# zertovitch/zip-ada

Measured on NVIDIA B200. Metric: bzip2_encode_MBps_900k, higher is better.
Workload: dtype u8

## Files before the change

zip-ada_b200/csrc/b2_api.cu:

```cuda
#include "b2_common.cuh"
#include "b2_kernels.h"
#include "../../include/b2gpu.h"

#include <algorithm>
#include <atomic>
#include <cmath>
#include <condition_variable>
#include <cstdlib>
#include <cstring>
#include <deque>
#include <chrono>
#include <map>
#include <mutex>
#include <string>
#include <thread>
#include <vector>
#include <unordered_set>

static thread_local std::string g_last_error = "";
void b2_set_error(const char *file, int line, const char *msg) {
  char buf[512];
  snprintf(buf, sizeof buf, "%s:%d: %s", file, line, msg);
  g_last_error = buf;
}
// ... 117 lines not shown
  DevBuf<u8> d_packed;
  DevBuf<u32> d_cut_first, d_cut_last, d_cut_tsum;
  DevBuf<u64> d_cut_carry, d_cut_tincl;
  DevBuf<u8> d_cut_gs;
  DevBuf<u16> d_cut_gm;
  DevBuf<B2ZipCrcTables> d_zt;
  DevBuf<B2ZipTile> d_ztiles;
  DevBuf<B2ZipEntry> d_zents;
  DevBuf<B2ZipCopy> d_zcopies;
  DevBuf<u32> d_zpartial, d_zcrc;
  DevBuf<u8> d_vstream, d_vlcol, d_vrle, d_vsel;
  DevBuf<u32> d_vlink, d_vchain, d_vscal;
  DevBuf<u64> d_vcand;
  DevBuf<B2VBlock> d_vblocks;
  std::vector<Workspace *> ws;
  std::vector<B2Chunk> chunks;
  std::vector<u32> nseg;
  std::vector<std::vector<u32>> seg;
  std::vector<b2_chunk_trace> trace;
  b2_stats stats;
  B2SortStats sort_stats;
  bool batch_positions_fixed = false;
  size_t batch_positions = 1536ull << 20;
  size_t first_batch_positions = ~(size_t)0;
  size_t batch_jobs_max = 65535;
  int n_workspaces = 1;
  u64 launches_other = 0;
  cudaEvent_t ev[2] = {nullptr, nullptr};
  cudaEvent_t ev_call[2] = {nullptr, nullptr};
};

namespace {

struct StageTimer {
  cudaStream_t st; cudaEvent_t *ev; double *acc; bool on;
  StageTimer(b2_encoder *e, cudaStream_t st_, cudaEvent_t *ev_, double *acc_) : st(st_), ev(ev_), acc(acc_), on(e->timing >= 2) {
    if (on) cudaEventRecord(ev[0], st);
  }
  ~StageTimer() {
    if (on) {
      cudaEventRecord(ev[1], st);
      cudaEventSynchronize(ev[1]);
      float ms = 0; cudaEventElapsedTime(&ms, ev[0], ev[1]);
      *acc += ms;
    }
  }
};

void balance_window(int level, i64 &lo, i64 &hi) {
  volatile float fcap = (float)(100000 * level);
  volatile float flo = fcap * 1.05f, fhi = fcap * 1.30f;
  lo = -1; hi = -2;
  i64 base = 100000ll * level;
  for (i64 v = base; v <= 2 * base; v++) {
    volatile float f = (float)v;
    if (f >= flo && f <= fhi) { if (lo < 0) lo = v; hi = v; }
  }
}

int ensure_batch_workspace(Workspace *w, size_t T, size_t J) {
  const size_t max_tiles = T / B2_SORT_TILE + J + 8;
  const size_t max_mtiles = T / B2_MTF_TILE + J + 8;
  const size_t GT = T / B2_GROUP_SIZE + 20 * J + 32;
  B2_TRY(w->d_scalars.ensure(16));
  B2_TRY(w->d_jobs.ensure(J));
  B2_TRY(w->d_text.ensure(T + 64)); B2_TRY(w->d_bwt.ensure(T + 64)); B2_TRY(w->d_idx.ensure(T + 64));
  B2_TRY(w->d_m16.ensure((T / 16 + 8 * J + 8) * 8)); B2_TRY(w->d_m256.ensure((T / 256 + 2 * J + 8) * 8));
  B2_TRY(w->d_keysA.ensure(T)); B2_TRY(w->d_keysB.ensure(T));
  B2_TRY(w->d_valsA.ensure(T)); B2_TRY(w->d_valsB.ensure(T));
  B2_TRY(w->d_rank.ensure(T)); B2_TRY(w->d_grp.ensure(T));
  B2_TRY(w->d_slotA.ensure(T)); B2_TRY(w->d_slotB.ensure(T)); B2_TRY(w->d_sa.ensure(T)); B2_TRY(w->d_tile_cnt.ensure(max_tiles));
  B2_TRY(w->d_tiles.ensure(max_tiles)); B2_TRY(w->d_tiles_rr.ensure(max_tiles)); B2_TRY(w->d_mtiles.ensure(max_mtiles));
  B2_TRY(w->d_tilemask.ensure(max_mtiles * 8)); B2_TRY(w->d_msegs.ensure(T / B2_MTF_SEG + J + 8));
  B2_TRY(w->d_sj.ensure(J));
  B2_TRY(w->d_hist.ensure(max_tiles * 256)); B2_TRY(w->d_digit_base.ensure(J * 8 * 256 + 256));
  B2_TRY(w->d_tile_head.ensure(max_tiles)); B2_TRY(w->d_carry.ensure(max_tiles));
  B2_TRY(w->d_unsorted.ensure(J));
  B2_TRY(w->d_mtf.ensure(T + 16 * J + 64)); B2_TRY(w->d_ghist.ensure(T + 16 * J + 64));
  B2_TRY(w->d_rank3.ensure(GT)); B2_TRY(w->d_rank4.ensure(GT)); B2_TRY(w->d_gdist.ensure(GT));
  B2_TRY(w->d_sel.ensure(GT * B2_N_TRIPLES + 64)); B2_TRY(w->d_selprev.ensure(GT * B2_N_TRIPLES + 64));
  B2_TRY(w->d_selpos.ensure(GT));
  B2_TRY(w->d_gpack.ensure(GT * B2_N_TRIPLES + 64)); B2_TRY(w->d_gselcost.ensure(GT * B2_N_TRIPLES + 64));
  B2_TRY(w->d_ehist.ensure(J * B2_N_TRIPLES * B2_MAX_CODERS * 260));
  B2_TRY(w->d_leaves.ensure((J * B2_N_TRIPLES * B2_MAX_CODERS + 64) * 260)); B2_TRY(w->d_wl.ensure(J * B2_N_TRIPLES * (B2_MAX_CODERS + 3) + J / 32 + 512));
  B2_TRY(w->d_estat.ensure(J * B2_N_TRIPLES * 2)); B2_TRY(w->d_selcost.ensure(J * B2_N_TRIPLES));
  B2_TRY(w->d_lens.ensure(J * B2_N_TRIPLES * B2_MAX_CODERS * B2_MAX_ALPHA));
  B2_TRY(w->d_cost.ensure(J * B2_N_TRIPLES)); B2_TRY(w->d_low.ensure(J * B2_N_TRIPLES));
  B2_TRY(w->d_items.ensure(J));
  if (J > w->h_unsorted_cap) {
    if (w->h_unsorted) cudaFreeHost(w->h_unsorted);
    B2_CUDA_CHECK(cudaMallocHost((void **)&w->h_unsorted, (J + 64) * sizeof(u32)));
    w->h_unsorted_cap = J + 64;
  }
  return 0;
}

u64 layout_jobs(std::vector<B2Job> &jobs, int level) {
  u64 pos = 0, mpos = 0;
  for (auto &j : jobs) {
    u64 cap = std::min<u64>((u64)j.raw_len * 5 / 4 + 8, (u64)level * 100000 + 64);
    cap = (cap + 255) & ~255ull;
    j.pos_off = (u32)pos; j.cap = (u32)cap;
    pos += cap;
    j.mtf_off = (u32)mpos;
    mpos += (cap + 2 + 7) & ~7ull;
  }
  return pos;
}

int run_batch(b2_encoder *e, Workspace *w, const u8 *d_in, std::vector<B2Job> &jobs) {
  const u32 J = (u32)jobs.size();
  if (J == 0) return 0;
  const u64 T = layout_jobs(jobs, e->level);
  if (T >= (1ull << 32) - (1ull << 20)) B2_FAIL(B2_ERR_INTERNAL, "batch too large for 32-bit arena offsets (lower B2GPU_BATCH_POSITIONS)");
  B2_TRY(ensure_batch_workspace(w, (size_t)T + 64, J));
  cudaStream_t st = w->st;
  B2_CUDA_CHECK(cudaMemcpyAsync(w->d_jobs.p, jobs.data(), J * sizeof(B2Job), cudaMemcpyHostToDevice, st));
  {
    StageTimer tm(e, st, w->ev, &w->stage_ms[1]);
    B2_TRY(b2k_rle1(st, d_in, w->d_jobs.p, J, w->d_text.p, e->d_ct.p));
    w->launches += 1;
  }
  w->batch_jobs.resize(J);
  B2_CUDA_CHECK(cudaMemcpyAsync(w->batch_jobs.data(), w->d_jobs.p, J * sizeof(B2Job), cudaMemcpyDeviceToHost, st));
  B2_CUDA_CHECK(cudaStreamSynchronize(st));
  u32 gpos = 0, max_g = 1;
  std::vector<u32> ids(J), ns(J);
  std::vector<B2SortTile> mtiles, msegs, msegs_mid, msegs_big;
  for (u32 j = 0; j < J; j++) {
    B2Job &b = w->batch_jobs[j];
    if (b.n > b.cap) B2_FAIL(B2_ERR_INTERNAL, "RLE1 output exceeds its slot");
    u32 gmax = (b.n / B2_GROUP_SIZE + 2 + 15) & ~15u;
    b.grp_off = gpos; gpos += gmax;
    max_g = std::max(max_g, gmax);
    ids[j] = j; ns[j] = b.n;
    b.na = b.n;
    b.tile0 = (u32)mtiles.size();
    for (u32 s = 0; s < b.n; s += B2_MTF_TILE) mtiles.push_back(B2SortTile{j, s});
    for (u32 s = 0; s < b.n; s += B2_MTF_SEG) (b.n_used <= 64 ? msegs : b.n_used <= 128 ? msegs_mid : msegs_big).push_back(B2SortTile{j, s});
    w->block_bytes += b.n;
  }
  w->blocks += J;
  w->total_groups = gpos;
  B2_CUDA_CHECK(cudaMemcpyAsync(w->d_jobs.p, w->batch_jobs.data(), J * sizeof(B2Job), cudaMemcpyHostToDevice, st));
  {
    StageTimer tm(e, st, w->ev, &w->stage_ms[2]);
    B2SortCtx cx;
    cx.keysA = w->d_keysA.p; cx.keysB = w->d_keysB.p; cx.valsA = w->d_valsA.p; cx.valsB = w->d_valsB.p;
    cx.rank = w->d_rank.p; cx.grp = w->d_grp.p; cx.d_tiles = w->d_tiles.p; cx.d_sj = w->d_sj.p;
    cx.slotA = w->d_slotA.p; cx.slotB = w->d_slotB.p; cx.sa_full = w->d_sa.p; cx.d_tile_cnt = w->d_tile_cnt.p;
    cx.d_hist = w->d_hist.p; cx.d_digit_base = w->d_digit_base.p; cx.d_tiles_rr = w->d_tiles_rr.p; cx.d_ticket = w->d_digit_base.p + w->d_digit_base.cap - 256; cx.d_tile_head = w->d_tile_head.p; cx.d_carry = w->d_carry.p;
    cx.d_unsorted = w->d_unsorted.p; cx.h_unsorted = w->h_unsorted;
    cx.max_tiles = w->d_tiles.cap; cx.max_jobs = w->d_sj.cap; cx.timing = e->timing >= 1;
    cx.stats = w->sort_stats;
    {
      u32 max_used = 1;
      for (u32 j = 0; j < J; j++) max_used = std::max(max_used, w->batch_jobs[j].n_used);
      cx.sym_bits = 1;
      while ((1u << cx.sym_bits) < max_used) cx.sym_bits++;
      cx.max_used = max_used;
      cx.h_jobs = w->batch_jobs.data();
    }
    if (e->timing >= 1) cudaEventRecord(w->ev_sort[0], st);
    int rc = b2k_bwt_batch(&cx, st, w->d_jobs.p, ids, ns, w->d_text.p, w->d_bwt.p);
    if (e->timing >= 1) cudaEventRecord(w->ev_sort[1], st);
    w->sort_stats = cx.stats;
    if (rc) return rc;
// ... 1326 lines not shown
```

zip-ada_b200/csrc/b2_entropy.cu:

```cuda
#include "b2_common.cuh"
#include "b2_kernels.h"

#define HSTRIDE 260
#define QS_SMALL 100

__global__ void __launch_bounds__(256)
k_group_keys(const B2Job *__restrict__ jobs, const u16 *__restrict__ mtf, u32 *__restrict__ rank3, u32 *__restrict__ rank4) {
  const B2Job &job = jobs[blockIdx.x];
  const u32 M = job.n_mtf, G = job.n_groups;
  const u16 *m = mtf + job.mtf_off;
  const u32 eob = job.n_used + 1;
  const u32 lim3 = eob < 3 ? eob : 3, lim4 = eob < 4 ? eob : 4;
  for (u32 g = threadIdx.x; g < G; g += blockDim.x) {
    u32 s0 = g * B2_GROUP_SIZE, s1 = min(s0 + B2_GROUP_SIZE, M);
    u32 k3 = 0, k4 = 0;
    for (u32 s = s0; s < s1; s++) { u32 sym = m[s]; k3 += sym < lim3; k4 += sym < lim4; }
    rank3[job.grp_off + g] = (k3 << 16) | (g + 1);
    rank4[job.grp_off + g] = (k4 << 16) | (g + 1);
  }
}

__global__ void __launch_bounds__(256)
k_group_hist(const B2Job *__restrict__ jobs, const u16 *__restrict__ mtf, u16 *__restrict__ ghist, u8 *__restrict__ gdist) {
  const B2Job &job = jobs[blockIdx.x];
// ... 32 lines not shown
    }
    cntA += addA;
    const bool newB = leadB && foundAt == 0xFFFFFFFFu;
    const u32 bmB = __ballot_sync(0xffffffffu, newB);
    u16 *e = gh + s0;
    if (leadA) e[slotA] = (u16)((cntA << 9) | symA);
    if (newB) e[DA + __popc(bmB & lt)] = (u16)((cntB << 9) | symB);
    if (l == 0) gdist[job.grp_off + g] = (u8)(DA + __popc(bmB));
  }
}

__global__ void __launch_bounds__(32)
k_rank_sort(const B2Job *__restrict__ jobs, u32 *__restrict__ rank3, u32 *__restrict__ rank4, u32 g_lo, u32 g_hi) {
  extern __shared__ __align__(16) u32 a[];
  const B2Job &job = jobs[blockIdx.x >> 1];
  u32 *arr = ((blockIdx.x & 1) ? rank4 : rank3) + job.grp_off;
  const i32 G = (i32)job.n_groups;
  if ((u32)G <= g_lo || (u32)G > g_hi) return;
  for (i32 i = threadIdx.x; i < G; i += 32) a[i + 1] = arr[i];
  __syncwarp();
  if (threadIdx.x == 0) {
    i32 mx = G;
    u32 temp;
#define KEY(x) ((x) >> 16)
    auto sift = [&](i32 s) {
      i32 c = s;
      while (8 * c + 7 <= mx) {
        const uint2 pr = *reinterpret_cast<const uint2 *>(&a[2 * c]);
        const uint4 qd = *reinterpret_cast<const uint4 *>(&a[4 * c]);
        const uint4 o0 = *reinterpret_cast<const uint4 *>(&a[8 * c]);
        const uint4 o1 = *reinterpret_cast<const uint4 *>(&a[8 * c + 4]);
        const bool r1 = KEY(pr.x) < KEY(pr.y);
        const i32 s1 = 2 * c + (r1 ? 1 : 0);
        const u32 g0 = r1 ? qd.z : qd.x, g1 = r1 ? qd.w : qd.y;
        const bool r2 = KEY(g0) < KEY(g1);
        const i32 s2 = 2 * s1 + (r2 ? 1 : 0);
        const u32 ox = r1 ? o1.x : o0.x, oy = r1 ? o1.y : o0.y, oz = r1 ? o1.z : o0.z, ow = r1 ? o1.w : o0.w;
        const u32 h0 = r2 ? oz : ox, h1 = r2 ? ow : oy;
        const bool r3 = KEY(h0) < KEY(h1);
        a[c] = r1 ? pr.y : pr.x;
        a[s1] = r2 ? g1 : g0;
        a[s2] = r3 ? h1 : h0;
        c = 2 * s2 + (r3 ? 1 : 0);
      }
      while (4 * c + 3 <= mx) {
        const uint2 pr = *reinterpret_cast<const uint2 *>(&a[2 * c]);
        const uint4 qd = *reinterpret_cast<const uint4 *>(&a[4 * c]);
        const bool r1 = KEY(pr.x) < KEY(pr.y);
        const i32 s1 = 2 * c + (r1 ? 1 : 0);
        const u32 g0 = r1 ? qd.z : qd.x, g1 = r1 ? qd.w : qd.y;
        const bool r2 = KEY(g0) < KEY(g1);
        a[c] = r1 ? pr.y : pr.x;
        a[s1] = r2 ? g1 : g0;
        c = 2 * s1 + (r2 ? 1 : 0);
      }
      for (;;) {
        i32 son = 2 * c;
        if (son > mx) break;
        if (son < mx && KEY(a[son]) < KEY(a[son + 1])) son++;
        a[c] = a[son];
        c = son;
      }
      while (c != s) {
        i32 father = c >> 1;
        if (KEY(a[father]) < KEY(temp)) { a[c] = a[father]; c = father; } else break;
      }
      a[c] = temp;
    };
    for (i32 j = mx / 2; j >= 1; j--) { temp = a[j]; sift(j); }
    while (mx > 1) {
      temp = a[mx];
      a[mx] = a[1];
      mx--;
      sift(1);
    }
#undef KEY
  }
  __syncwarp();
  for (i32 i = threadIdx.x; i < G; i += 32) arr[i] = a[i + 1];
}

struct EntArgs {
  const B2Job *jobs;
  const u16 *mtf;
  const u16 *ghist;
  const u8 *gdist;
  const u32 *rank3, *rank4;
  u8 *sel, *selprev;
  u32 *gpack;
  u16 *gselcost;
  u32 *hist;
  u32 *leaves;
  u32 *wl, *wl_count;
  u32 *wl_off;
  u32 *chg;
  u32 *pl, *pl_count;
  u8 *lens;
  u32 *stat;
  u32 *selcost;
  u32 *cost_all, *low_all;
  u32 total_groups;
  int level, n_triples;
  u32 n_jobs;
};

__host__ __device__ inline u32 b2_choice_mask(int level, u32 M) {
  if (level == 9) {
    if (M <= 5000) return (1u << 2) | (1u << 3) | (1u << 6);
    if (M <= 10000) return (1u << 3) | (1u << 4) | (1u << 6);
    return (1u << 3) | (1u << 4) | (1u << 5) | (1u << 6);
  }
  return (1u << 4) | (1u << 6);
}

__device__ __forceinline__ size_t leaf_index(u32 q, u32 e) { return ((size_t)(q >> 5) * HSTRIDE + e) * 32 + (q & 31); }

__global__ void __launch_bounds__(256)
k_ent_init(EntArgs a) {
  const int t = blockIdx.x;
  const u32 jb = blockIdx.y;
  const B2Job &job = a.jobs[jb];
  const u32 G = job.n_groups;
  int max_len, sw, ec;
  b2_triple(a.level, t, max_len, sw, ec);
  const u32 p = jb * B2_N_TRIPLES + t;
  u8 *sel = a.sel + (size_t)t * a.total_groups + job.grp_off;
  u8 *selprev = a.selprev + (size_t)t * a.total_groups + job.grp_off;
  const u32 *rk = (sw == 3 ? a.rank3 : a.rank4) + job.grp_off;
  const int attr_tab[5][6] = {{2, 1, 0, 0, 0, 0}, {3, 1, 2, 0, 0, 0}, {4, 2, 1, 3, 0, 0}, {5, 3, 1, 2, 4, 0}, {6, 4, 2, 1, 3, 5}};
  for (u32 i = threadIdx.x; i < G; i += 256) {
    const u32 pos1 = i + 1;
    int r = 1;
    while ((u64)r * G / ec < pos1) r++;
    sel[(rk[i] & 0xFFFFu) - 1] = (u8)attr_tab[ec - 2][r - 1];
    selprev[i] = 0;
  }
  u32 *h = a.hist + (size_t)p * (B2_MAX_CODERS * HSTRIDE);
  for (u32 i = threadIdx.x; i < B2_MAX_CODERS * HSTRIDE; i += 256) h[i] = 0;
  u8 *ln = a.lens + (size_t)p * B2_MAX_CODERS * B2_MAX_ALPHA;
  for (u32 i = threadIdx.x; i < B2_MAX_CODERS * B2_MAX_ALPHA; i += 256) ln[i] = 0;
  if (threadIdx.x == 0) {
    const bool always = (b2_choice_mask(a.level, job.n_mtf) >> ec) & 1u;
    a.stat[2 * p] = 1;
    a.stat[2 * p + 1] = always ? 0u : 2u;
    a.chg[p] = 0x80000000u;
  }
}

#define WL_TILE 2048
__device__ __forceinline__ u32 wl_items(const EntArgs &a, u32 p) {
  const int t = (int)(p % B2_N_TRIPLES);
  if (p >= a.n_jobs * B2_N_TRIPLES || t >= a.n_triples || a.stat[2 * p + 1] != 0) return 0;
  return (u32)__popc(a.chg[p] & 63u) | 0x10000u;
}
__global__ void __launch_bounds__(1024)
k_ent_wl_sum(EntArgs a, u32 *tile_sum) {
  __shared__ u32 sm[40];
  const u32 p = blockIdx.x * WL_TILE + 2 * threadIdx.x;
  u32 total;
  block_excl_add(wl_items(a, p) + wl_items(a, p + 1), sm, &total);
  if (threadIdx.x == 0) { tile_sum[2 * blockIdx.x] = total & 0xFFFFu; tile_sum[2 * blockIdx.x + 1] = total >> 16; }
}
__global__ void __launch_bounds__(1024)
k_ent_wl_scan(EntArgs a, const u32 *tile_sum) {
  __shared__ u32 sm[40];
  u32 before_c = 0, before_p = 0;
  for (u32 b = threadIdx.x; b < blockIdx.x; b += 1024) { before_c += tile_sum[2 * b]; before_p += tile_sum[2 * b + 1]; }
  u32 base_c, base_p;
  block_excl_add(before_c, sm, &base_c);
  __syncthreads();
  block_excl_add(before_p, sm, &base_p);
  __syncthreads();
  const u32 P = a.n_jobs * B2_N_TRIPLES;
  const u32 p = blockIdx.x * WL_TILE + 2 * threadIdx.x;
  const u32 c0 = wl_items(a, p), c1 = wl_items(a, p + 1);
  u32 total;
  const u32 ex = block_excl_add(c0 + c1, sm, &total);
  if (p < P) { a.wl_off[p] = base_c + (ex & 0xFFFFu); if (c0 >> 16) a.pl[base_p + (ex >> 16)] = p; }
  if (p + 1 < P) { a.wl_off[p + 1] = base_c + ((ex + c0) & 0xFFFFu); if (c1 >> 16) a.pl[base_p + ((ex + c0) >> 16)] = p + 1; }
  if (blockIdx.x == gridDim.x - 1 && threadIdx.x == 0) { *a.wl_count = base_c + (total & 0xFFFFu); *a.pl_count = base_p + (total >> 16); }
}

__global__ void __launch_bounds__(256)
k_ent_hist(EntArgs a) {
  __shared__ u32 h[B2_MAX_CODERS][HSTRIDE];
  __shared__ u32 changed;
  const int t = blockIdx.x;
  const u32 jb = blockIdx.y;
  const u32 p = jb * B2_N_TRIPLES + t;
  if (a.stat[2 * p + 1]) return;
  const B2Job &job = a.jobs[jb];
  const u32 G = job.n_groups;
  int max_len, sw, ec;
  b2_triple(a.level, t, max_len, sw, ec);
  const u8 *sel = a.sel + (size_t)t * a.total_groups + job.grp_off;
  u8 *selprev = a.selprev + (size_t)t * a.total_groups + job.grp_off;
  u32 *hg = a.hist + (size_t)p * (B2_MAX_CODERS * HSTRIDE);
  const u32 tid = threadIdx.x;
  for (u32 i = tid; i < (u32)ec * HSTRIDE; i += 256) (&h[0][0])[i] = hg[i];
  if (tid == 0) changed = 0;
  __syncthreads();
  const u16 *gh = a.ghist + job.mtf_off;
  const u8 *gd = a.gdist + job.grp_off;
  u32 mych = 0;
  for (u32 g = tid; g < G; g += 256) {
    const u32 c = sel[g], o = selprev[g];
    if (c == o) continue;
    const u16 *e = gh + g * B2_GROUP_SIZE;
    const u32 D = gd[g];
    for (u32 k = 0; k < D; k++) {
      const u32 v = e[k], sym = v & 511u, cn = v >> 9;
      atomicAdd(&h[c - 1][sym], cn);
      if (o) atomicSub(&h[o - 1][sym], cn);
    }
    mych |= (1u << (c - 1)) | (o ? (1u << (o - 1)) : 0u);
    selprev[g] = (u8)c;
  }
  mych = __reduce_or_sync(0xffffffffu, mych);
  if (lane_id() == 0 && mych) atomicOr(&changed, mych);
  __syncthreads();
  for (u32 i = tid; i < (u32)ec * HSTRIDE; i += 256) hg[i] = (&h[0][0])[i];
  if (tid == 0) a.chg[p] = (a.chg[p] & 0x80000000u) ? ((1u << ec) - 1u) : changed;
}
// ... 32 lines not shown
  const u32 slot = blockIdx.x * 32 + l;
  const u32 count = min(*a.wl_count, nq);
  if (blockIdx.x * 32 >= count) return;
  u32 n = 0;
  if (slot < count) {
    const u32 q = a.wl[slot];
    const u32 jb = (q / B2_MAX_CODERS) / B2_N_TRIPLES;
    n = a.jobs[jb].n_used + 2;
  }
  const u32 nmax = __reduce_max_sync(0xffffffffu, n);
  if (nmax <= n_lo || nmax > n_hi) return;
  u32 *g = a.leaves + (size_t)blockIdx.x * HSTRIDE * 32;
  for (u32 e = 0; e < nmax; e++) s[e * 32 + l] = g[e * 32 + l];
  __syncwarp();
#define EL(x) s[(x) * 32 + l]
  enum { SI = 1, SJ = 2, CK = 3 };
  int sp = 0, st = SI;
  u32 f = 0, nn = n, pw = 0;
  i32 i = 0, j = (i32)n - 1;
  bool active = n >= 2;
  if (active) pw = EL(nn / 2) >> 9;
  while (__any_sync(0xffffffffu, active)) {
    if (active) {
      if (st == SI) {
#pragma unroll
        for (int u = 0; u < 4; u++) { if (st == SI) { if ((EL(f + i) >> 9) < pw) i++; else st = SJ; } }
      }
      if (st == SJ) {
#pragma unroll
        for (int u = 0; u < 4; u++) { if (st == SJ) { if (pw < (EL(f + j) >> 9)) j--; else st = CK; } }
      }
      if (st == CK) {
        if (i >= j) {
          const u32 n1 = (u32)i, n2 = nn - (u32)i;
          u32 fa = f, na = n1, fb = f + (u32)i, nb = n2;
          if (n1 > n2) { fa = f + (u32)i; na = n2; fb = f; nb = n1; }
          if (na < 2) { fa = fb; na = nb; nb = 0; }
          if (nb >= 2) stk[(sp++) * 32 + l] = (fb << 16) | nb;
          if (na < 2) {
            if (sp == 0) active = false;
            else { const u32 v = stk[(--sp) * 32 + l]; fa = v >> 16; na = v & 0xFFFFu; }
          }
          if (active) {
            f = fa; nn = na;
            pw = EL(f + nn / 2) >> 9;
            i = 0; j = (i32)nn - 1;
          }
        } else {
          const u32 x = EL(f + i), y = EL(f + j);
          EL(f + i) = y; EL(f + j) = x;
          i++; j--;
        }
        st = SI;
      }
    }
  }
#undef EL
  __syncwarp();
  for (u32 e = 0; e < nmax; e++) g[e * 32 + l] = s[e * 32 + l];
}

#include "b2_pm.cuh"

__global__ void __launch_bounds__(32 * PM_WARPS)
k_ent_pm(EntArgs a, u32 nq, u32 alpha_max, int variant) {
  extern __shared__ u32 pm_smem[];
  const u32 w = warp_id(), l = lane_id();
  const u32 slot = blockIdx.x * PM_WARPS + w;
  if (slot >= min(*a.wl_count, nq)) return;
  LLScratch S = ll_scratch_at(pm_smem + (size_t)w * ll_scratch_words(alpha_max), alpha_max);
  const u32 q = a.wl[slot];
  const u32 p = q / B2_MAX_CODERS, c = q % B2_MAX_CODERS;
  const u32 jb = p / B2_N_TRIPLES, t = p % B2_N_TRIPLES;
  int max_len, sw, ec;
  b2_triple(a.level, (int)t, max_len, sw, ec);
  const int ns = (int)a.jobs[jb].n_used + 2;
  for (int e = l; e < ns; e += 32) S.leaf[e] = a.leaves[leaf_index(slot, (u32)e)];
  __syncwarp();
  u8 *lens = a.lens + ((size_t)p * B2_MAX_CODERS + c) * B2_MAX_ALPHA;
  if (variant == 0) ll_package_merge_warp(S, ns, max_len, lens);
  else ll_package_merge_warp_mp(S, ns, max_len, lens);
}

__global__ void __launch_bounds__(256)
k_ent_cost(EntArgs a) {
  __shared__ unsigned long long lenpack[HSTRIDE];
  const int t = blockIdx.x;
  const u32 jb = blockIdx.y;
  const u32 p = jb * B2_N_TRIPLES + t;
  if (a.stat[2 * p + 1]) return;
  const B2Job &job = a.jobs[jb];
  const u32 M = job.n_mtf, G = job.n_groups;
  const int A = (int)job.n_used + 2;
  const u16 *m = a.mtf + job.mtf_off;
  int max_len, sw, ec;
  b2_triple(a.level, t, max_len, sw, ec);
  const u8 *lens = a.lens + (size_t)p * B2_MAX_CODERS * B2_MAX_ALPHA;
  for (int s = threadIdx.x; s < A; s += 256) {
    unsigned long long v = 0;
    for (int c = 0; c < ec; c++) v |= (unsigned long long)lens[c * B2_MAX_ALPHA + s] << (10 * c);
    lenpack[s] = v;
  }
  __syncthreads();
  u32 *gpack = a.gpack + (size_t)t * a.total_groups + job.grp_off;
  u16 *gselcost = a.gselcost + (size_t)t * a.total_groups + job.grp_off;
  const u8 *sel = a.sel + (size_t)t * a.total_groups + job.grp_off;
  const u16 *gh = a.ghist + job.mtf_off;
  const u8 *gd = a.gdist + job.grp_off;
  __shared__ u32 rows[8][32 * B2_GROUP_SIZE / 2];
  const u32 wid = threadIdx.x >> 5, ln = threadIdx.x & 31u;
  const u32 *gh32 = reinterpret_cast<const u32 *>(gh);
  for (u32 gb = 0; gb < G; gb += 256) {
    const u32 gw = gb + 32 * wid;
    const u32 nrow = gw < G ? min(32u, G - gw) : 0u;
    __syncwarp();
    for (u32 i = ln; i < nrow * (B2_GROUP_SIZE / 2); i += 32) rows[wid][i] = gh32[(size_t)gw * (B2_GROUP_SIZE / 2) + i];
    __syncwarp();
    const u32 g = gw + ln;
    if (g >= G) continue;
    const u32 *e2 = rows[wid] + ln * (B2_GROUP_SIZE / 2);
    const u32 D = gd[g];
    unsigned long long acc = 0;
    for (u32 k = 0; k + 1 < D; k += 2) {
      const u32 v = e2[k >> 1];
      acc += lenpack[v & 511u] * (unsigned long long)((v >> 9) & 127u);
      acc += lenpack[(v >> 16) & 511u] * (unsigned long long)(v >> 25);
    }
    if (D & 1u) { const u32 v = e2[D >> 1] & 0xFFFFu; acc += lenpack[v & 511u] * (unsigned long long)(v >> 9); }
    u32 c[6], mn = 0xFFFFFFFFu;
#pragma unroll
    for (int cl = 0; cl < 6; cl++) { c[cl] = (u32)((acc >> (10 * cl)) & 1023u); if (cl < ec) mn = min(mn, c[cl]); }
    u32 pk = 0;
#pragma unroll
    for (int cl = 0; cl < 6; cl++) pk |= (cl < ec ? min(c[cl] - mn, 7u) : 7u) << (4 * cl);
    gpack[g] = pk;
    const u32 sc = sel[g] - 1;
    u32 mine = c[0];
#pragma unroll
    for (int cl = 1; cl < 6; cl++) mine = (sc == (u32)cl) ? c[cl] : mine;
    gselcost[g] = (u16)mine;
  }
}

__global__ void __launch_bounds__(32)
k_ent_sweep(EntArgs a) {
  const u32 slot = blockIdx.x * 32 + threadIdx.x;
  const u32 count = *a.pl_count;
  if (blockIdx.x * 32 >= count) return;
  const bool active = slot < count;
  const u32 p = a.pl[active ? slot : blockIdx.x * 32];
  const u32 jb = p / B2_N_TRIPLES, t = p % B2_N_TRIPLES;
  const B2Job &job = a.jobs[jb];
  const u32 G = active ? job.n_groups : 0u;
  const u32 Gmax = __reduce_max_sync(0xffffffffu, G);
  int max_len, sw, ec;
  b2_triple(a.level, (int)t, max_len, sw, ec);
  const size_t base = (size_t)t * a.total_groups + job.grp_off;
  const u32 *gc = a.gpack + base;
  u8 *sel = a.sel + base;
  u32 posv = 0;
#pragma unroll
  for (int cl = 0; cl < 6; cl++) posv |= (cl < ec ? (u32)cl + 1u : 7u) << (4 * cl);
  u32 def = 0;
  u32 nx[16];
  u32 ns[4] = {0, 0, 0, 0};
  auto load16g = [&](u32 g0) {
#pragma unroll
    for (int k = 0; k < 16; k++) nx[k] = 0;
    ns[0] = ns[1] = ns[2] = ns[3] = 0;
    if (g0 < G) {
#pragma unroll
      for (int k = 0; k < 4; k++) {
        const uint4 x = *reinterpret_cast<const uint4 *>(gc + g0 + 4 * k);
        nx[4 * k] = x.x; nx[4 * k + 1] = x.y; nx[4 * k + 2] = x.z; nx[4 * k + 3] = x.w;
      }
      const uint4 sv = *reinterpret_cast<const uint4 *>(sel + g0);
      ns[0] = sv.x; ns[1] = sv.y; ns[2] = sv.z; ns[3] = sv.w;
      if (g0 + 256 < G) asm volatile("prefetch.global.L2 [%0];" ::"l"(gc + g0 + 256));
    }
  };
  load16g(0);
  for (u32 g0 = 0; g0 < Gmax; g0 += 16) {
    u32 c16[16];
#pragma unroll
    for (int k = 0; k < 16; k++) c16[k] = nx[k];
    const u32 s4[4] = {ns[0], ns[1], ns[2], ns[3]};
    load16g(g0 + 16);
#pragma unroll
    for (int k = 0; k < 16; k++) {
      if (g0 + k < G) {
        const u32 clk = (s4[k >> 2] >> (8 * (k & 3))) & 255u;
        const u32 sum = c16[k] + posv;
        const u32 ev = ((sum & 0x000F0F0Fu) << 3) | 0x00040200u;
        const u32 od = (((sum >> 4) & 0x000F0F0Fu) << 3) | 0x00050301u;
        const u32 m3 = __vminu4(ev, od);
        const u32 key = min(min(m3 & 255u, (m3 >> 8) & 255u), (m3 >> 16) & 255u);
        const u32 best0 = key & 7u;
        if (best0 + 1 != clk) { def++; sel[g0 + k] = (u8)(best0 + 1); }
        const u32 pl = (posv >> (4 * best0)) & 15u;
        posv += (~(posv + (8u - pl) * 0x111111u) & 0x888888u) >> 3;
        posv = (posv & ~(15u << (4 * best0))) | (1u << (4 * best0));
      }
    }
  }
  if (active) { a.stat[2 * p] = def; if (def == 0) a.stat[2 * p + 1] = 1; }
}

__global__ void __launch_bounds__(32)
k_ent_selcost(EntArgs a) {
  const u32 jb = blockIdx.x;
  const u32 t = threadIdx.x;
  const B2Job &job = a.jobs[jb];
  const u32 G = job.n_groups;
  const bool active = (int)t < a.n_triples;
  const u8 *sel = a.sel + (size_t)(active ? t : 0) * a.total_groups + job.grp_off;
  u32 posv = 0x654321u;
  u32 bits = 0;
  uint4 nx = *reinterpret_cast<const uint4 *>(sel);
  for (u32 g0 = 0; g0 < G; g0 += 16) {
    const uint4 cur = nx;
    if (g0 + 16 < G) nx = *reinterpret_cast<const uint4 *>(sel + g0 + 16);
    const u32 w4[4] = {cur.x, cur.y, cur.z, cur.w};
#pragma unroll
    for (int k = 0; k < 16; k++) {
      if (g0 + k < G) {
        const u32 cl0 = ((w4[k >> 2] >> (8 * (k & 3))) & 255u) - 1;
        const u32 pl = (posv >> (4 * cl0)) & 15u;
        bits += pl;
        posv += (~(posv + (8u - pl) * 0x111111u) & 0x888888u) >> 3;
        posv = (posv & ~(15u << (4 * cl0))) | (1u << (4 * cl0));
      }
    }
  }
  if (active) a.selcost[jb * B2_N_TRIPLES + t] = bits;
}

__global__ void __launch_bounds__(256)
k_ent_final(EntArgs a) {
  __shared__ u32 stat[8];
  __shared__ u32 red[8];
  const int t = blockIdx.x;
  const u32 jb = blockIdx.y;
  const u32 p = jb * B2_N_TRIPLES + t;
  if (a.stat[2 * p + 1] == 2u) return;
  const B2Job &job = a.jobs[jb];
  const u32 G = job.n_groups;
  const int A = (int)job.n_used + 2;
  int max_len, sw, ec;
  b2_triple(a.level, t, max_len, sw, ec);
  const u8 *lens = a.lens + (size_t)p * B2_MAX_CODERS * B2_MAX_ALPHA;
  const u8 *sel = a.sel + (size_t)t * a.total_groups + job.grp_off;
  const u16 *gselcost = a.gselcost + (size_t)t * a.total_groups + job.grp_off;
  const u32 tid = threadIdx.x;
  if (tid < 8) stat[tid] = 0;
  __syncthreads();
  u32 part = 0;
  for (u32 g = tid; g < G; g += 256) {
    const u32 c = sel[g];
    atomicAdd(&stat[c], 1u);
    part += gselcost[g];
  }
  for (int i = tid; i < ec * A; i += 256) {
    const int c = i / A, s = i % A;
    const int cur = s == 0 ? lens[c * B2_MAX_ALPHA] : lens[c * B2_MAX_ALPHA + s - 1];
    const int nw = lens[c * B2_MAX_ALPHA + s];
    const int dlt = nw > cur ? nw - cur : cur - nw;
    part += 2 * dlt + 1 + (s == 0 ? 5 : 0);
  }
#pragma unroll
  for (int o = 16; o; o >>= 1) part += __shfl_xor_sync(0xffffffffu, part, o);
  if (lane_id() == 0) red[warp_id()] = part;
  __syncthreads();
  if (tid == 0) {
    u32 total = a.selcost[p];
    for (int w = 0; w < 8; w++) total += red[w];
    const u32 uniform_usage = G / (u32)ec;
    u32 low = 0;
    for (int c = 1; c <= ec; c++) if (stat[c] < uniform_usage / 2) low = 1;
    a.cost_all[p] = total;
    a.low_all[p] = low;
    a.stat[2 * p + 1] = 1;
  }
}

__global__ void k_ent_gate(EntArgs a, u32 *activated) {
  const u32 jb = blockIdx.x * blockDim.x + threadIdx.x;
  if (jb >= a.n_jobs) return;
  const u32 mask = b2_choice_mask(a.level, a.jobs[jb].n_mtf);
  u32 count = 0;
  for (int t0 = 0; t0 < a.n_triples; t0 += 5) {
    bool low = false;
    bool known = true;
    for (int c = 0; c < 5 && known; c++) {
      const int ec = 6 - c;
      const u32 p = jb * B2_N_TRIPLES + t0 + c;
      const bool runs = low || ((mask >> ec) & 1u);
      if (!runs) continue;
      const u32 f = a.stat[2 * p + 1];
      if (f == 2u) { a.stat[2 * p + 1] = 0; count++; known = false; }
      else low = a.low_all[p] != 0;
    }
  }
  if (count) atomicAdd(activated, count);
}

__global__ void k_choose(B2Job *jobs, u32 n_jobs, const u32 *__restrict__ cost_all, const u32 *__restrict__ low_all,
                         int level, int n_triples) {
  u32 jb = blockIdx.x * blockDim.x + threadIdx.x;
  if (jb >= n_jobs) return;
  B2Job &job = jobs[jb];
  const u32 M = job.n_mtf;
  const u32 choice_mask = b2_choice_mask(level, M);
  bool low = false;
  u32 best_cost = 0x7FFFFFFFu, best = 0;
  for (int t = 0; t < n_triples; t++) {
    int max_len, sw, ec;
    b2_triple(level, t, max_len, sw, ec);
    if (low || ((choice_mask >> ec) & 1u)) {
      u32 cost = cost_all[(size_t)jb * B2_N_TRIPLES + t];
      low = low_all[(size_t)jb * B2_N_TRIPLES + t] != 0;
      if (cost < best_cost) { best_cost = cost; best = (u32)t; }
    }
  }
  job.best = best;
  job.best_cost = best_cost;
  u32 ranges = 0;
  for (int i = 0; i < 16; i++) {
    u32 wv = job.in_use[i >> 1];
    u32 h = (i & 1) ? (wv >> 16) : (wv & 0xFFFFu);
    if (h) ranges++;
  }
  job.nbits = 105ull + 16ull + 16ull * ranges + 3ull + 15ull + (u64)best_cost;
}

int b2k_entropy(cudaStream_t st, B2Job *d_jobs, u32 n_jobs, u32 max_groups_per_job, u32 total_groups,
                const u16 *d_mtf, u16 *d_ghist, u8 *d_gdist, u32 *d_rank3, u32 *d_rank4, u8 *d_sel, u8 *d_selprev,
                u32 *d_gpack, u16 *d_gselcost,
                u32 *d_hist, u32 *d_leaves, u32 *d_wl, u8 *d_lens, u32 *d_stat, u32 *d_selcost, u32 *d_cost, u32 *d_low,
                int level, u32 max_alpha, u32 *d_activated, u64 *launches) {
  B2_CUDA_CHECK(cudaFuncSetAttribute(k_rank_sort, cudaFuncAttributeMaxDynamicSharedMemorySize, 18064 * 4));
  B2_CUDA_CHECK(cudaFuncSetAttribute(k_ent_qsort, cudaFuncAttributeMaxDynamicSharedMemorySize, (HSTRIDE + 16) * 32 * 4));
  if (n_jobs == 0) return 0;
  if (max_alpha < 2) max_alpha = 2;
  if (max_alpha > HSTRIDE) max_alpha = HSTRIDE;
  const size_t qs_smem = ((size_t)max_alpha + 16) * 32 * 4;
  const size_t pm_smem = (size_t)PM_WARPS * ll_scratch_words(max_alpha) * 4;
  int pm_variant = 1;
  if (const char *e = getenv("B2GPU_PM")) pm_variant = atoi(e) ? 1 : 0;
  const int n_triples = level == 9 ? 20 : 5;
  k_group_keys<<<n_jobs, 256, 0, st>>>(d_jobs, d_mtf, d_rank3, d_rank4);
  k_group_hist<<<n_jobs, 256, 0, st>>>(d_jobs, d_mtf, d_ghist, d_gdist);
  {
    u32 lo = 0;
    for (u32 hi = 2304; lo < max_groups_per_job; hi *= 2) {
      const u32 top = hi >= max_groups_per_job ? max_groups_per_job : hi;
      k_rank_sort<<<n_jobs * 2, 32, ((size_t)top + 2) * 4, st>>>(d_jobs, d_rank3, d_rank4, lo, top);
      *launches += 1;
      lo = top;
    }
  }
  EntArgs a;
  a.jobs = d_jobs; a.mtf = d_mtf; a.ghist = d_ghist; a.gdist = d_gdist; a.rank3 = d_rank3; a.rank4 = d_rank4; a.sel = d_sel; a.selprev = d_selprev;
  a.gpack = d_gpack; a.gselcost = d_gselcost; a.hist = d_hist; a.leaves = d_leaves; a.wl = d_wl; a.wl_count = d_activated + 1; a.pl_count = d_activated + 2; a.wl_off = d_wl + (size_t)n_jobs * B2_N_TRIPLES * B2_MAX_CODERS + 32;
  a.chg = a.wl_off + (size_t)n_jobs * B2_N_TRIPLES + 32; a.pl = a.chg + (size_t)n_jobs * B2_N_TRIPLES + 32; a.lens = d_lens; a.stat = d_stat; a.selcost = d_selcost;
  a.cost_all = d_cost; a.low_all = d_low; a.total_groups = total_groups; a.level = level; a.n_triples = n_triples;
  a.n_jobs = n_jobs;
  const dim3 grid(n_triples, n_jobs);
  const u32 nq = n_jobs * B2_N_TRIPLES * B2_MAX_CODERS;
  const u32 wl_tiles = (n_jobs * B2_N_TRIPLES + WL_TILE - 1) / WL_TILE;
  u32 *wl_tile_sum = a.pl + (size_t)n_jobs * B2_N_TRIPLES + 32;
  const u32 np = n_jobs * B2_N_TRIPLES;
  k_ent_init<<<grid, 256, 0, st>>>(a);
  *launches += 4;
  for (int phase = 0; phase < 4; phase++) {
    for (int it = 0; it <= 10; it++) {
      k_ent_hist<<<grid, 256, 0, st>>>(a);
      k_ent_wl_sum<<<wl_tiles, 1024, 0, st>>>(a, wl_tile_sum);
      k_ent_wl_scan<<<wl_tiles, 1024, 0, st>>>(a, wl_tile_sum);
      k_ent_leaves<<<grid, 256, 0, st>>>(a);
      if (max_alpha > QS_SMALL) {
        k_ent_qsort<<<(nq + 31) / 32, 32, ((size_t)QS_SMALL + 16) * 32 * 4, st>>>(a, nq, QS_SMALL, 0, QS_SMALL);
        k_ent_qsort<<<(nq + 31) / 32, 32, qs_smem, st>>>(a, nq, max_alpha, QS_SMALL, HSTRIDE);
        *launches += 1;
      } else {
        k_ent_qsort<<<(nq + 31) / 32, 32, qs_smem, st>>>(a, nq, max_alpha, 0, HSTRIDE);
      }
      k_ent_pm<<<(nq + PM_WARPS - 1) / PM_WARPS, 32 * PM_WARPS, pm_smem, st>>>(a, nq, max_alpha, pm_variant);
      k_ent_cost<<<grid, 256, 0, st>>>(a);
      *launches += 7;
      if (it < 10) { k_ent_sweep<<<(np + 31) / 32, 32, 0, st>>>(a); *launches += 1; }
    }
    k_ent_selcost<<<n_jobs, 32, 0, st>>>(a);
    k_ent_final<<<grid, 256, 0, st>>>(a);
    B2_CUDA_CHECK(cudaMemsetAsync(d_activated, 0, sizeof(u32), st));
    k_ent_gate<<<(n_jobs + 127) / 128, 128, 0, st>>>(a, d_activated);
    *launches += 3;
    u32 activated = 0;
    B2_CUDA_CHECK(cudaMemcpyAsync(&activated, d_activated, sizeof(u32), cudaMemcpyDeviceToHost, st));
    B2_CUDA_CHECK(cudaStreamSynchronize(st));
    if (!activated) break;
  }
  k_choose<<<(n_jobs + 127) / 128, 128, 0, st>>>(d_jobs, n_jobs, d_cost, d_low, level, n_triples);
  *launches += 3;
  B2_CUDA_CHECK(cudaGetLastError());
  return 0;
}
```

Baseline: 1833.

## Parallelize selector sweep across warp lanes and tile cost kernel over triples

The sequential per-triple selector sweep becomes warp-parallel for large jobs. Each lane handles a chunk of groups, starting from a cached or warmed-up MTF-position state, and chunks are re-run until each lane's starting state matches its predecessor's ending state. The cost kernel now tiles groups across blocks and evaluates four active triples per pass with 32-bit packed lengths, so each ghist row is loaded once for all triples rather than once per triple. This adds a per-triple predecessor-state buffer, possible extra re-run passes, and a tighter 5-bit packing whose sums could overflow if costs grow large.

```diff
diff --git a/zip-ada_b200/csrc/b2_api.cu b/zip-ada_b200/csrc/b2_api.cu
--- a/zip-ada_b200/csrc/b2_api.cu
+++ b/zip-ada_b200/csrc/b2_api.cu
@@ -223,7 +223,7 @@
   B2_TRY(w->d_selpos.ensure(GT));
   B2_TRY(w->d_gpack.ensure(GT * B2_N_TRIPLES + 64)); B2_TRY(w->d_gselcost.ensure(GT * B2_N_TRIPLES + 64));
   B2_TRY(w->d_ehist.ensure(J * B2_N_TRIPLES * B2_MAX_CODERS * 260));
-  B2_TRY(w->d_leaves.ensure((J * B2_N_TRIPLES * B2_MAX_CODERS + 64) * 260)); B2_TRY(w->d_wl.ensure(J * B2_N_TRIPLES * (B2_MAX_CODERS + 3) + J / 32 + 512));
+  B2_TRY(w->d_leaves.ensure((J * B2_N_TRIPLES * B2_MAX_CODERS + 64) * 260)); B2_TRY(w->d_wl.ensure(J * B2_N_TRIPLES * (B2_MAX_CODERS + 3 + 32) + J / 32 + 512));
   B2_TRY(w->d_estat.ensure(J * B2_N_TRIPLES * 2)); B2_TRY(w->d_selcost.ensure(J * B2_N_TRIPLES));
   B2_TRY(w->d_lens.ensure(J * B2_N_TRIPLES * B2_MAX_CODERS * B2_MAX_ALPHA));
   B2_TRY(w->d_cost.ensure(J * B2_N_TRIPLES)); B2_TRY(w->d_low.ensure(J * B2_N_TRIPLES));
diff --git a/zip-ada_b200/csrc/b2_entropy.cu b/zip-ada_b200/csrc/b2_entropy.cu
--- a/zip-ada_b200/csrc/b2_entropy.cu
+++ b/zip-ada_b200/csrc/b2_entropy.cu
@@ -138,7 +138,6 @@
 
 struct EntArgs {
   const B2Job *jobs;
-  const u16 *mtf;
   const u16 *ghist;
   const u8 *gdist;
   const u32 *rank3, *rank4;
@@ -153,6 +152,7 @@
   u32 *pl, *pl_count;
   u8 *lens;
   u32 *stat;
+  u32 *pred;
   u32 *selcost;
   u32 *cost_all, *low_all;
   u32 total_groups;
@@ -195,6 +195,7 @@
   for (u32 i = threadIdx.x; i < B2_MAX_CODERS * HSTRIDE; i += 256) h[i] = 0;
   u8 *ln = a.lens + (size_t)p * B2_MAX_CODERS * B2_MAX_ALPHA;
   for (u32 i = threadIdx.x; i < B2_MAX_CODERS * B2_MAX_ALPHA; i += 256) ln[i] = 0;
+  if (threadIdx.x < 32) a.pred[(size_t)p * 32 + threadIdx.x] = 0;
   if (threadIdx.x == 0) {
     const bool always = (b2_choice_mask(a.level, job.n_mtf) >> ec) & 1u;
     a.stat[2 * p] = 1;
@@ -393,129 +394,103 @@
   else ll_package_merge_warp_mp(S, ns, max_len, lens);
 }
 
+#define COST_TILE 2048
+#define COST_TC 4
+#define LP_EVEN 0x01F07C1Fu
 __global__ void __launch_bounds__(256)
 k_ent_cost(EntArgs a) {
-  __shared__ unsigned long long lenpack[HSTRIDE];
-  const int t = blockIdx.x;
+  __shared__ u32 lenpack[B2_N_TRIPLES][HSTRIDE];
+  __shared__ u32 rows[8][32 * B2_GROUP_SIZE / 2];
+  __shared__ u32 tlist[B2_N_TRIPLES];
+  __shared__ u32 n_act;
   const u32 jb = blockIdx.y;
-  const u32 p = jb * B2_N_TRIPLES + t;
-  if (a.stat[2 * p + 1]) return;
   const B2Job &job = a.jobs[jb];
-  const u32 M = job.n_mtf, G = job.n_groups;
-  const int A = (int)job.n_used + 2;
-  const u16 *m = a.mtf + job.mtf_off;
-  int max_len, sw, ec;
-  b2_triple(a.level, t, max_len, sw, ec);
-  const u8 *lens = a.lens + (size_t)p * B2_MAX_CODERS * B2_MAX_ALPHA;
-  for (int s = threadIdx.x; s < A; s += 256) {
-    unsigned long long v = 0;
-    for (int c = 0; c < ec; c++) v |= (unsigned long long)lens[c * B2_MAX_ALPHA + s] << (10 * c);
-    lenpack[s] = v;
-  }
-  __syncthreads();
-  u32 *gpack = a.gpack + (size_t)t * a.total_groups + job.grp_off;
-  u16 *gselcost = a.gselcost + (size_t)t * a.total_groups + job.grp_off;
-  const u8 *sel = a.sel + (size_t)t * a.total_groups + job.grp_off;
+  const u32 G = job.n_groups;
+  const u32 gt0 = blockIdx.x * COST_TILE;
+  if (gt0 >= G) return;
+  const u32 wid = threadIdx.x >> 5, ln = threadIdx.x & 31u;
+  if (wid == 0) {
+    const u32 p = jb * B2_N_TRIPLES + ln;
+    const bool act = (int)ln < a.n_triples && a.stat[2 * p + 1] == 0;
+    const u32 m = __ballot_sync(0xffffffffu, act);
+    if (act) {
+      int max_len, sw, ec;
+      b2_triple(a.level, (int)ln, max_len, sw, ec);
+      tlist[__popc(m & ((1u << ln) - 1u))] = ln | ((u32)ec << 8);
+    }
+    if (ln == 0) n_act = __popc(m);
+  }
+  __syncthreads();
+  const u32 nact = n_act;
+  if (nact == 0) return;
+  const u32 npad = (nact + COST_TC - 1) / COST_TC * COST_TC;
+  const u32 A = job.n_used + 2;
+  for (u32 i = threadIdx.x; i < npad * A; i += 256) {
+    const u32 k = i / A, s = i % A;
+    u32 v = 0;
+    if (k < nact) {
+      const u32 t = tlist[k] & 255u, ec = tlist[k] >> 8;
+      const u8 *lens = a.lens + (size_t)(jb * B2_N_TRIPLES + t) * B2_MAX_CODERS * B2_MAX_ALPHA;
+      for (u32 c = 0; c < ec; c++) v |= (u32)lens[c * B2_MAX_ALPHA + s] << (5 * (c & 1) + 10 * (c >> 1));
+    }
+    lenpack[k][s] = v;
+  }
+  __syncthreads();
   const u16 *gh = a.ghist + job.mtf_off;
   const u8 *gd = a.gdist + job.grp_off;
-  __shared__ u32 rows[8][32 * B2_GROUP_SIZE / 2];
-  const u32 wid = threadIdx.x >> 5, ln = threadIdx.x & 31u;
   const u32 *gh32 = reinterpret_cast<const u32 *>(gh);
-  for (u32 gb = 0; gb < G; gb += 256) {
+  const u32 gend = min(G, gt0 + COST_TILE);
+  for (u32 gb = gt0; gb < gend; gb += 256) {
     const u32 gw = gb + 32 * wid;
-    const u32 nrow = gw < G ? min(32u, G - gw) : 0u;
+    const u32 nrow = gw < gend ? min(32u, gend - gw) : 0u;
     __syncwarp();
     for (u32 i = ln; i < nrow * (B2_GROUP_SIZE / 2); i += 32) rows[wid][i] = gh32[(size_t)gw * (B2_GROUP_SIZE / 2) + i];
     __syncwarp();
     const u32 g = gw + ln;
-    if (g >= G) continue;
+    if (g >= gend) continue;
     const u32 *e2 = rows[wid] + ln * (B2_GROUP_SIZE / 2);
     const u32 D = gd[g];
-    unsigned long long acc = 0;
-    for (u32 k = 0; k + 1 < D; k += 2) {
-      const u32 v = e2[k >> 1];
-      acc += lenpack[v & 511u] * (unsigned long long)((v >> 9) & 127u);
-      acc += lenpack[(v >> 16) & 511u] * (unsigned long long)(v >> 25);
-    }
-    if (D & 1u) { const u32 v = e2[D >> 1] & 0xFFFFu; acc += lenpack[v & 511u] * (unsigned long long)(v >> 9); }
-    u32 c[6], mn = 0xFFFFFFFFu;
-#pragma unroll
-    for (int cl = 0; cl < 6; cl++) { c[cl] = (u32)((acc >> (10 * cl)) & 1023u); if (cl < ec) mn = min(mn, c[cl]); }
-    u32 pk = 0;
-#pragma unroll
-    for (int cl = 0; cl < 6; cl++) pk |= (cl < ec ? min(c[cl] - mn, 7u) : 7u) << (4 * cl);
-    gpack[g] = pk;
-    const u32 sc = sel[g] - 1;
-    u32 mine = c[0];
-#pragma unroll
-    for (int cl = 1; cl < 6; cl++) mine = (sc == (u32)cl) ? c[cl] : mine;
-    gselcost[g] = (u16)mine;
-  }
-}
-
-__global__ void __launch_bounds__(32)
-k_ent_sweep(EntArgs a) {
-  const u32 slot = blockIdx.x * 32 + threadIdx.x;
-  const u32 count = *a.pl_count;
-  if (blockIdx.x * 32 >= count) return;
-  const bool active = slot < count;
-  const u32 p = a.pl[active ? slot : blockIdx.x * 32];
-  const u32 jb = p / B2_N_TRIPLES, t = p % B2_N_TRIPLES;
-  const B2Job &job = a.jobs[jb];
-  const u32 G = active ? job.n_groups : 0u;
-  const u32 Gmax = __reduce_max_sync(0xffffffffu, G);
-  int max_len, sw, ec;
-  b2_triple(a.level, (int)t, max_len, sw, ec);
-  const size_t base = (size_t)t * a.total_groups + job.grp_off;
-  const u32 *gc = a.gpack + base;
-  u8 *sel = a.sel + base;
-  u32 posv = 0;
-#pragma unroll
-  for (int cl = 0; cl < 6; cl++) posv |= (cl < ec ? (u32)cl + 1u : 7u) << (4 * cl);
-  u32 def = 0;
-  u32 nx[16];
-  u32 ns[4] = {0, 0, 0, 0};
-  auto load16g = [&](u32 g0) {
-#pragma unroll
-    for (int k = 0; k < 16; k++) nx[k] = 0;
-    ns[0] = ns[1] = ns[2] = ns[3] = 0;
-    if (g0 < G) {
-#pragma unroll
-      for (int k = 0; k < 4; k++) {
-        const uint4 x = *reinterpret_cast<const uint4 *>(gc + g0 + 4 * k);
-        nx[4 * k] = x.x; nx[4 * k + 1] = x.y; nx[4 * k + 2] = x.z; nx[4 * k + 3] = x.w;
-      }
-      const uint4 sv = *reinterpret_cast<const uint4 *>(sel + g0);
-      ns[0] = sv.x; ns[1] = sv.y; ns[2] = sv.z; ns[3] = sv.w;
-      if (g0 + 256 < G) asm volatile("prefetch.global.L2 [%0];" ::"l"(gc + g0 + 256));
-    }
-  };
-  load16g(0);
-  for (u32 g0 = 0; g0 < Gmax; g0 += 16) {
-    u32 c16[16];
-#pragma unroll
-    for (int k = 0; k < 16; k++) c16[k] = nx[k];
-    const u32 s4[4] = {ns[0], ns[1], ns[2], ns[3]};
-    load16g(g0 + 16);
-#pragma unroll
-    for (int k = 0; k < 16; k++) {
-      if (g0 + k < G) {
-        const u32 clk = (s4[k >> 2] >> (8 * (k & 3))) & 255u;
-        const u32 sum = c16[k] + posv;
-        const u32 ev = ((sum & 0x000F0F0Fu) << 3) | 0x00040200u;
-        const u32 od = (((sum >> 4) & 0x000F0F0Fu) << 3) | 0x00050301u;
-        const u32 m3 = __vminu4(ev, od);
-        const u32 key = min(min(m3 & 255u, (m3 >> 8) & 255u), (m3 >> 16) & 255u);
-        const u32 best0 = key & 7u;
-        if (best0 + 1 != clk) { def++; sel[g0 + k] = (u8)(best0 + 1); }
-        const u32 pl = (posv >> (4 * best0)) & 15u;
-        posv += (~(posv + (8u - pl) * 0x111111u) & 0x888888u) >> 3;
-        posv = (posv & ~(15u << (4 * best0))) | (1u << (4 * best0));
-      }
-    }
-  }
-  if (active) { a.stat[2 * p] = def; if (def == 0) a.stat[2 * p + 1] = 1; }
-}
+    for (u32 k0 = 0; k0 < nact; k0 += COST_TC) {
+      u32 ae[COST_TC], ao[COST_TC];
+#pragma unroll
+      for (int j = 0; j < COST_TC; j++) ae[j] = ao[j] = 0;
+      for (u32 k = 0; k < D; k += 2) {
+        const u32 v = e2[k >> 1], w = k + 1 < D ? v >> 16 : 0u;
+        const u32 s0 = v & 511u, c0 = (v >> 9) & 127u, s1 = w & 511u, c1 = w >> 9;
+#pragma unroll
+        for (int j = 0; j < COST_TC; j++) {
+          const u32 l0 = lenpack[k0 + j][s0], l1 = lenpack[k0 + j][s1];
+          ae[j] += (l0 & LP_EVEN) * c0 + (l1 & LP_EVEN) * c1;
+          ao[j] += ((l0 >> 5) & LP_EVEN) * c0 + ((l1 >> 5) & LP_EVEN) * c1;
+        }
+      }
+#pragma unroll
+      for (int j = 0; j < COST_TC; j++) {
+        if (k0 + j < nact) {
+          const u32 t = tlist[k0 + j] & 255u, ec = tlist[k0 + j] >> 8;
+          const size_t base = (size_t)t * a.total_groups + job.grp_off;
+          u32 c[6], mn = 0xFFFFFFFFu;
+#pragma unroll
+          for (int cl = 0; cl < 6; cl++) {
+            c[cl] = ((cl & 1 ? ao[j] : ae[j]) >> (10 * (cl >> 1))) & 1023u;
+            if ((u32)cl < ec) mn = min(mn, c[cl]);
+          }
+          u32 pk = 0;
+#pragma unroll
+          for (int cl = 0; cl < 6; cl++) pk |= ((u32)cl < ec ? min(c[cl] - mn, 7u) : 7u) << (4 * cl);
+          a.gpack[base + g] = pk;
+          const u32 sc = a.sel[base + g] - 1;
+          u32 mine = c[0];
+#pragma unroll
+          for (int cl = 1; cl < 6; cl++) mine = (sc == (u32)cl) ? c[cl] : mine;
+          a.gselcost[base + g] = (u16)mine;
+        }
+      }
+    }
+  }
+}
+
+#include "b2_sweep.cuh"
 
 __global__ void __launch_bounds__(32)
 k_ent_selcost(EntArgs a) {
@@ -671,7 +646,7 @@
     }
   }
   EntArgs a;
-  a.jobs = d_jobs; a.mtf = d_mtf; a.ghist = d_ghist; a.gdist = d_gdist; a.rank3 = d_rank3; a.rank4 = d_rank4; a.sel = d_sel; a.selprev = d_selprev;
+  a.jobs = d_jobs; a.ghist = d_ghist; a.gdist = d_gdist; a.rank3 = d_rank3; a.rank4 = d_rank4; a.sel = d_sel; a.selprev = d_selprev;
   a.gpack = d_gpack; a.gselcost = d_gselcost; a.hist = d_hist; a.leaves = d_leaves; a.wl = d_wl; a.wl_count = d_activated + 1; a.pl_count = d_activated + 2; a.wl_off = d_wl + (size_t)n_jobs * B2_N_TRIPLES * B2_MAX_CODERS + 32;
   a.chg = a.wl_off + (size_t)n_jobs * B2_N_TRIPLES + 32; a.pl = a.chg + (size_t)n_jobs * B2_N_TRIPLES + 32; a.lens = d_lens; a.stat = d_stat; a.selcost = d_selcost;
   a.cost_all = d_cost; a.low_all = d_low; a.total_groups = total_groups; a.level = level; a.n_triples = n_triples;
@@ -680,6 +655,11 @@
   const u32 nq = n_jobs * B2_N_TRIPLES * B2_MAX_CODERS;
   const u32 wl_tiles = (n_jobs * B2_N_TRIPLES + WL_TILE - 1) / WL_TILE;
   u32 *wl_tile_sum = a.pl + (size_t)n_jobs * B2_N_TRIPLES + 32;
+  a.pred = wl_tile_sum + 2 * (size_t)wl_tiles + 32;
+  SweepArgs sa;
+  sa.jobs = d_jobs; sa.pl = a.pl; sa.pl_count = a.pl_count; sa.gpack = d_gpack; sa.selprev = d_selprev; sa.sel = d_sel;
+  sa.stat = d_stat; sa.pred = a.pred; sa.total_groups = total_groups; sa.level = level;
+  const dim3 cost_grid((max_groups_per_job + COST_TILE - 1) / COST_TILE, n_jobs);
   const u32 np = n_jobs * B2_N_TRIPLES;
   k_ent_init<<<grid, 256, 0, st>>>(a);
   *launches += 4;
@@ -697,9 +677,9 @@
         k_ent_qsort<<<(nq + 31) / 32, 32, qs_smem, st>>>(a, nq, max_alpha, 0, HSTRIDE);
       }
       k_ent_pm<<<(nq + PM_WARPS - 1) / PM_WARPS, 32 * PM_WARPS, pm_smem, st>>>(a, nq, max_alpha, pm_variant);
-      k_ent_cost<<<grid, 256, 0, st>>>(a);
+      k_ent_cost<<<cost_grid, 256, 0, st>>>(a);
       *launches += 7;
-      if (it < 10) { k_ent_sweep<<<(np + 31) / 32, 32, 0, st>>>(a); *launches += 1; }
+      if (it < 10) { k_ent_sweep<<<(np + SWEEP_WARPS - 1) / SWEEP_WARPS, 32 * SWEEP_WARPS, 0, st>>>(sa); *launches += 1; }
     }
     k_ent_selcost<<<n_jobs, 32, 0, st>>>(a);
     k_ent_final<<<grid, 256, 0, st>>>(a);
diff --git a/zip-ada_b200/csrc/b2_sweep.cuh b/zip-ada_b200/csrc/b2_sweep.cuh
--- /dev/null
+++ b/zip-ada_b200/csrc/b2_sweep.cuh
@@ -0,0 +1,135 @@
+#pragma once
+#include "b2_common.cuh"
+
+#define SWEEP_LANE_MAX 512
+#define SWEEP_WARMUP 64
+#define SWEEP_WARPS 4
+#define SWEEP_PRED_OK 0x80000000u
+
+struct SweepArgs {
+  const B2Job *jobs;
+  const u32 *pl, *pl_count;
+  const u32 *gpack;
+  const u8 *selprev;
+  u8 *sel;
+  u32 *stat;
+  u32 *pred;
+  u32 total_groups;
+  int level;
+};
+
+__host__ __device__ inline u32 sweep_posv0(int ec) {
+  u32 posv = 0;
+  for (int cl = 0; cl < 6; cl++) posv |= (cl < ec ? (u32)cl + 1u : 7u) << (4 * cl);
+  return posv;
+}
+
+__device__ __forceinline__ u32 sweep_run(const u32 *__restrict__ gc, const u8 *__restrict__ old, u8 *__restrict__ sel,
+                                         u32 g0, u32 g1, u32 posv, u32 &def, int mode) {
+  u32 nx[16];
+  u32 ns[4] = {0, 0, 0, 0};
+  auto load16g = [&](u32 g) {
+    if (g < g1) {
+#pragma unroll
+      for (int k = 0; k < 4; k++) {
+        const uint4 x = *reinterpret_cast<const uint4 *>(gc + g + 4 * k);
+        nx[4 * k] = x.x; nx[4 * k + 1] = x.y; nx[4 * k + 2] = x.z; nx[4 * k + 3] = x.w;
+      }
+      if (mode) { const uint4 sv = *reinterpret_cast<const uint4 *>(old + g); ns[0] = sv.x; ns[1] = sv.y; ns[2] = sv.z; ns[3] = sv.w; }
+#ifndef B2_EMU
+      if (g + 256 < g1) asm volatile("prefetch.global.L2 [%0];" ::"l"(gc + g + 256));
+#endif
+    }
+  };
+  load16g(g0);
+  for (u32 g = g0; g < g1; g += 16) {
+    u32 c16[16];
+#pragma unroll
+    for (int k = 0; k < 16; k++) c16[k] = nx[k];
+    const u32 s4[4] = {ns[0], ns[1], ns[2], ns[3]};
+    load16g(g + 16);
+#pragma unroll
+    for (int k = 0; k < 16; k++) {
+      if (g + k < g1) {
+        const u32 sum = c16[k] + posv;
+        const u32 ev = ((sum & 0x000F0F0Fu) << 3) | 0x00040200u;
+        const u32 od = (((sum >> 4) & 0x000F0F0Fu) << 3) | 0x00050301u;
+        const u32 m3 = __vminu4(ev, od);
+        const u32 key = min(min(m3 & 255u, (m3 >> 8) & 255u), (m3 >> 16) & 255u);
+        const u32 best0 = key & 7u;
+        if (mode) {
+          const u32 clk = (s4[k >> 2] >> (8 * (k & 3))) & 255u;
+          if (best0 + 1 != clk) def++;
+          if (best0 + 1 != clk || mode == 2) sel[g + k] = (u8)(best0 + 1);
+        }
+        const u32 pl = (posv >> (4 * best0)) & 15u;
+        posv += (~(posv + (8u - pl) * 0x111111u) & 0x888888u) >> 3;
+        posv = (posv & ~(15u << (4 * best0))) | (1u << (4 * best0));
+      }
+    }
+  }
+  return posv;
+}
+
+__device__ __forceinline__ u32 sweep_warp(const u32 *__restrict__ gc, const u8 *__restrict__ old, u8 *__restrict__ sel,
+                                          u32 *__restrict__ pred, u32 G, int ec) {
+  const u32 l = lane_id();
+  const u32 S = ((G + 31) / 32 + 15) & ~15u;
+  const u32 g0 = l * S, g1 = min(G, g0 + S);
+  const bool has = g0 < G;
+  const u32 posv0 = sweep_posv0(ec);
+  u32 start = posv0, end = 0, def = 0;
+  if (has && l > 0) {
+    const u32 pv = pred[l];
+    if (pv & SWEEP_PRED_OK) start = pv & 0xFFFFFFu;
+    else start = sweep_run(gc, old, sel, g0 - min(g0, (u32)SWEEP_WARMUP), g0, posv0, def, 0);
+  }
+  if (has) end = sweep_run(gc, old, sel, g0, g1, start, def, 1);
+  for (;;) {
+    const u32 prev = __shfl_up_sync(0xffffffffu, end, 1);
+    const bool bad = has && l > 0 && prev != start;
+    if (!__ballot_sync(0xffffffffu, bad)) break;
+    if (bad) {
+      start = prev;
+      def = 0;
+      end = sweep_run(gc, old, sel, g0, g1, start, def, 2);
+    }
+  }
+  if (has) pred[l] = start | SWEEP_PRED_OK;
+  return __reduce_add_sync(0xffffffffu, def);
+}
+
+__global__ void __launch_bounds__(32 * SWEEP_WARPS)
+k_ent_sweep(SweepArgs a) {
+  const u32 count = *a.pl_count;
+  const u32 slot = blockIdx.x * SWEEP_WARPS + warp_id();
+  if (slot >= count) return;
+  {
+    const u32 p = a.pl[slot];
+    const u32 jb = p / B2_N_TRIPLES, t = p % B2_N_TRIPLES;
+    const B2Job &job = a.jobs[jb];
+    const u32 G = job.n_groups;
+    if (G > SWEEP_LANE_MAX) {
+      int max_len, sw, ec;
+      b2_triple(a.level, (int)t, max_len, sw, ec);
+      const size_t base = (size_t)t * a.total_groups + job.grp_off;
+      const u32 def = sweep_warp(a.gpack + base, a.selprev + base, a.sel + base, a.pred + (size_t)p * 32, G, ec);
+      if (lane_id() == 0) { a.stat[2 * p] = def; if (def == 0) a.stat[2 * p + 1] = 1; }
+    }
+  }
+  if (slot % 32 == 0 && slot + lane_id() < count) {
+    const u32 p = a.pl[slot + lane_id()];
+    const u32 jb = p / B2_N_TRIPLES, t = p % B2_N_TRIPLES;
+    const B2Job &job = a.jobs[jb];
+    const u32 G = job.n_groups;
+    if (G <= SWEEP_LANE_MAX) {
+      int max_len, sw, ec;
+      b2_triple(a.level, (int)t, max_len, sw, ec);
+      const size_t base = (size_t)t * a.total_groups + job.grp_off;
+      u32 def = 0;
+      sweep_run(a.gpack + base, a.selprev + base, a.sel + base, 0, G, sweep_posv0(ec), def, 1);
+      a.stat[2 * p] = def;
+      if (def == 0) a.stat[2 * p + 1] = 1;
+    }
+  }
+}
```

Result: faster. 1943 (median of 6 runs) (+6.0%).
